# UW-RoboSoccer/tsid_control

Hardware: AMD Instinct MI355X
Metric: env-steps/sec (whole node) (higher is better)
Workload: dtype f64

## Files before the change

tsid_control_amd/csrc/tsidb_api.hip:

```cpp
#include "../../include/tsidb.h"
#include "tsidb_common.hpp"
#include "tsidb_sim.hpp"
#include "tsidb_tick.hpp"
#include "tsidb_policy.hpp"

#include <cmath>
#include <cstdio>
#include <cstring>
#include <string>
#include <vector>

using namespace tsidb;

template <typename T>
struct WalkArgs {
  const T *coef; const int *side; const int *nsteps; const T *rest; const T *com; int K;
  T t_now; const T *t_off; T Tstep, t_start, omega, z0, dz;
  const T *frames; T *foot_ref; T *contact_ref; uint8_t *cact; T *com_ref;
  const int *ncon; const int *con; int *latch; unsigned long long fgeoms0, fgeoms1; T td_frac; const double *t_dev;
};
template <typename T>
__device__ __forceinline__ void walk_update_env(const WalkArgs<T> &wa, int e, int r) {
  const T *coef = wa.coef, *rest = wa.rest, *com = wa.com, *t_off = wa.t_off, *frames = wa.frames;
  const int *side = wa.side, *nsteps = wa.nsteps, *ncon = wa.ncon, *con = wa.con;
// ... 170 lines not shown
  for (int b = 0; b < (MULTI ? B : 1); b++) {
    const DevModel<T> *mq = mp;
    if constexpr (MULTI) {
      asm volatile("" : "+s"(mq), "+s"(qpos), "+s"(qvel), "+s"(qacc_ws), "+s"(env_params), "+s"(terrain), "+s"(motor_tau) : : "memory");
      asm volatile("" : "+s"(qacc), "+s"(ncon), "+s"(con), "+s"(info) : : "memory");
      if constexpr (XF) asm volatile("" : "+s"(xfrc) : : "memory");
      if constexpr (RO) asm volatile("" : "+s"(ro.con_force), "+s"(ro.con_frame), "+s"(ro.con_pos), "+s"(ro.act_force), "+s"(ro.foot_grf) : : "memory");
      if constexpr (SE) asm volatile("" : "+s"(ro.sens) : : "memory");
      if constexpr (CT) asm volatile("" : "+s"(ctrl) : : "memory");
    }
    SimOut<T> roe{};
    if constexpr (RO) {
      roe.con_force = ro.con_force ? ro.con_force + E * MAXCON * 6 : nullptr;
      roe.con_frame = ro.con_frame ? ro.con_frame + E * MAXCON * 9 : nullptr;
      roe.con_pos = ro.con_pos ? ro.con_pos + E * MAXCON * 4 : nullptr;
      roe.act_force = ro.act_force ? ro.act_force + E * NA : nullptr;
      roe.foot_grf = ro.foot_grf ? ro.foot_grf + E * 12 : nullptr;
      roe.foot_body[0] = ro.foot_body[0]; roe.foot_body[1] = ro.foot_body[1];
    }
    if constexpr (SE) roe.sens = ro.sens + E * NSENS * mq->nsite;
    const size_t slot = (size_t)((ring.slots >> (4 * b)) & 15ull);
    const T *q_tsid = ring.q ? ring.q + slot * (size_t)n * NQ : nullptr, *v_tsid = ring.v ? ring.v + slot * (size_t)n * NV : nullptr;
    bool skip;
    {
      T chk = 0, big = 0;
      if (lane < NQ) { big += fabs(qpos[E * NQ + lane]); chk += q_tsid ? fabs(q_tsid[E * NQ + lane]) : T(0); }
      if (lane < NV) { big += fabs(qvel[E * NV + lane]); chk += fabs(qacc_ws[E * NV + lane]) + (v_tsid ? fabs(v_tsid[E * NV + lane]) : T(0)); }
      if (lane < NA && motor_tau) chk += fabs(motor_tau[E * NA + lane]);
      if constexpr (XF) for (int i = lane; i < NB * 6; i += WAVE) chk += fabs(xfrc[E * NB * 6 + i]);
      if constexpr (CT) { if (lane < NA) chk += fabs(ctrl[E * NA + lane]); }
      big = wave_sum(big);
      skip = __ballot(!(chk <= Eps<T>::inf)) || !(big <= T(SIM_STATE_BOUND));
      if (skip && wv == 0) {
        if (lane == 0) {
          if (info) { info[E * 4 + 2] = 0; info[E * 4 + 3] = 4; }
          if (ncon) ncon[e] = 0;
        }
        if (con && lane < MAXCON) con[E * MAXCON + lane] = -1;
        if constexpr (RO) sim_readouts_zero(roe, lane);
        if constexpr (SE) sim_sensors_zero(*mq, roe.sens, lane);
      }
    }
    if (!skip)
      sim_step_env<T, NW, XF, RO, SE, CT>(*mq, L, lane, wv, q_tsid ? q_tsid + E * NQ : nullptr, v_tsid ? v_tsid + E * NV : nullptr, qpos + E * NQ, qvel + E * NV, qacc_ws + E * NV,
                          env_params ? env_params + E * 8 : nullptr, terrain ? terrain + E * 20 : nullptr, XF ? xfrc + E * NB * 6 : nullptr,
                          motor_tau ? motor_tau + E * NA : nullptr, qacc ? qacc + E * NV : nullptr, ncon ? ncon + e : nullptr, con ? con + E * MAXCON : nullptr,
                          info ? info + E * 4 : nullptr, roe, CT ? ctrl + E * NA : nullptr, ctrl_mode);
    if constexpr (MULTI) __syncthreads();
  }
}

template <typename T>
__global__ __launch_bounds__(WAVE) void k_rbd(const DevModel<T> *__restrict__ mp, int n, const T *q, const T *v, T *M, T *hb,
                                              T *Jcom, T *Jf, T *oMf, T *com) {
  __shared__ TickLds<T> L;
  const int lane = threadIdx.x;
  if ((int)blockIdx.x >= n) return;
  const int e = env_of_block(blockIdx.x, n);
  const size_t E = (size_t)e;
  if (lane < NQ) L.qs[lane] = q[E * NQ + lane];
  if (lane < NV) L.vs[lane] = v[E * NV + lane];
  __syncthreads();
  rbd_terms<T>(*mp, L, lane);
  for (int i = lane; i < NV * NV; i += WAVE) M[E * NV * NV + i] = L.Dyn[(i / NV) * LDD + i % NV];
  if (lane < NV) hb[E * NV + lane] = L.h[lane];
  for (int i = lane; i < 3 * NV; i += WAVE) Jcom[E * 3 * NV + i] = L.k.Jcom[(i / NV) * LDF + i % NV];
  for (int i = lane; i < 12 * NV; i += WAVE) Jf[E * 12 * NV + i] = L.k.Jf[(i / NV) * LDF + i % NV];
// ... 505 lines not shown
  if ((int)ct[8] != CONDIM) throw std::string("model blob: contact dimension differs from this library's");
  const double *dmp = b.f64("mj_damping", NV), *ar = b.f64("mj_act_range", NA * 4);
  bool anyd = false;
  for (int i = 0; i < NV; i++) { m.mj_damping[i] = (T)dmp[i]; anyd |= dmp[i] != 0.0; }
  if (anyd != EULERDAMP) throw std::string("model blob: joint damping differs from what this library was built for");
  for (int i = 0; i < NA * 4; i++) {
    const double lim = sizeof(T) == 8 ? 1e300 : 1e30;
    m.act_range[i / 4][i % 4] = (T)(ar[i] > lim ? lim : (ar[i] < -lim ? -lim : ar[i]));
  }
  for (int i = 0; i < 7; i++) m.opt[i] = (T)op[i];
  m.opt[0] = (T)P[P_DT];
  m.opt[6] = sizeof(T) == 8 ? (T)1e-9 : (T)2e-6;
  for (int i = 0; i < 12; i++) m.contact[i] = (T)ct[i];
  const uint32_t nvert = h->blob.count("mj_hull_vert") / 3;
  m.hull_x = (const T *)h->d_hull;
  m.hull_y = m.hull_x + nvert;
  m.hull_z = m.hull_y + nvert;
  {
    const uint32_t np2 = b.count("mj_pairs");
    if (np2 % 2 || np2 / 2 > MAXPAIR) throw std::string("model blob: too many candidate body pairs");
    const int *pp = b.i32("mj_pairs", 0);
    m.npair = (int)(np2 / 2);
    for (int k = 0; k < m.npair; k++) {
      m.pair_a[k] = pp[2 * k]; m.pair_b[k] = pp[2 * k + 1];
      if (pp[2 * k] < 0 || pp[2 * k] >= NG || pp[2 * k + 1] < 0 || pp[2 * k + 1] >= NG) throw std::string("model blob: bad geom pair");
    }
    const double *hc = b.f64("mj_hull_center", NG * 3), *hb = b.f64("mj_hull_box", NG * 6);
    for (int i = 0; i < NG * 3; i++) m.hcen[i / 3][i % 3] = (T)hc[i];
    for (int i = 0; i < NG * 6; i++) m.hbox[i / 6][i % 6] = (T)hb[i];
    if (sizeof(T) == 4) for (int j = 0; j < NG; j++) for (int i = 3; i < 6; i++) m.hbox[j][i] = m.hbox[j][i] * (T)1.00001 + (T)1e-7;
  }
  memcpy(m.chunk_adr, b.i32("mj_chunk_adr", NG + 1), sizeof m.chunk_adr);
  m.chunk_box = (const T *)h->d_box;
  m.hull_eadr = h->d_eadr;
  m.hull_edge = h->d_edge;
  m.nsite = h->n_sites;
  for (int s = 0; s < h->n_sites; s++) {
    m.site_body[s] = h->site_body[s];
    for (int i = 0; i < 3; i++) m.site_pos[s][i] = (T)h->site_pos[s][i];
    for (int i = 0; i < 9; i++) m.site_R[s][i] = (T)h->site_R[s][i];
  }
}

static void validate_geometry(const Blob &b) {
  if constexpr (!TOPO_HAS_SIM) return;
  const int *ha = b.i32("mj_hull_adr", NG + 1), *ca = b.i32("mj_chunk_adr", NG + 1);
  const int64_t nvert = b.count("mj_hull_vert") / 3, nchunk = b.count("mj_chunk_box") / 6, nedge = b.count("mj_hull_edge");
  if (b.count("mj_hull_vert") % 3 || b.count("mj_chunk_box") % 6) throw std::string("model blob: hull vertex / chunk box sections are not whole records");
// ... 615 lines not shown
  need_refs(h);
  if (!q || !v || !tau || !dv || !f || !status) throw std::string("tsidb_tick_walk: null buffer");
  launch_tick(h, q, v, tau, dv, f, status, obs, obs_ld, frames, info, (hipStream_t)stream, nullptr, nullptr, walk, q_snapshot, v_snapshot);
  GUARD_END
}

int tsidb_rbd_terms(tsidb_handle h, const void *q, const void *v, void *M, void *hbias, void *Jcom, void *Jf, void *oMf,
                    void *com, void *stream) {
  GUARD_BEGIN
  if (!q || !v || !M || !hbias || !Jcom || !Jf || !oMf || !com) throw std::string("tsidb_rbd_terms: null buffer");
  hipStream_t s = (hipStream_t)stream;
  h->note_stream(s);
  with_dtype(h->dtype, [&](auto t) {
    using T = decltype(t);
    hipLaunchKernelGGL(k_rbd<T>, dim3(h->num_envs), dim3(WAVE), 0, s, (const DevModel<T> *)h->d_model, h->num_envs, (const T *)q,
                       (const T *)v, (T *)M, (T *)hbias, (T *)Jcom, (T *)Jf, (T *)oMf, (T *)com);
  });
  HIP_OK(hipGetLastError());
  GUARD_END
}

#ifdef TSIDB_STAMPS
int tsidb_debug_stamps(unsigned long long *out, int n) {
  return (int)hipMemcpyFromSymbol(out, HIP_SYMBOL(g_stamp), sizeof(unsigned long long) * 32 * (size_t)n);
}
#endif

int tsidb_dims(int *out9) {
  if (!out9) return -1;
  const int d[9] = {NJ, NQ, NV, NA, NB, TOPO_HAS_SIM, NG, CONDIM, TOPO_EULERDAMP};
  for (int i = 0; i < 9; i++) out9[i] = d[i];
  return 0;
}

int tsidb_lds_bytes(int dtype, int which) {
  return with_dtype(dtype, [&](auto t) { return which == 0 ? (int)sizeof(TickLds<decltype(t)>) : (int)sizeof(SimLds<decltype(t)>); });
}

}
```

tsid_control_amd/csrc/tsidb_common.hpp:

```cpp
#pragma once
#include <hip/hip_runtime.h>
#include <stdint.h>

#ifdef TSIDB_STAMPS
__device__ unsigned long long g_stamp[8192][32];
#define TSIDB_STAMP(k) do { if (threadIdx.x == 0 && blockIdx.x < 8192) g_stamp[blockIdx.x][k] = __builtin_amdgcn_s_memtime(); } while (0)
#define TSIDB_LAP_INIT() unsigned long long lap_t_ = __builtin_amdgcn_s_memtime()
#define TSIDB_LAP(k) do { unsigned long long n_ = __builtin_amdgcn_s_memtime(); if (threadIdx.x == 0 && blockIdx.x < 8192) g_stamp[blockIdx.x][k] += n_ - lap_t_; lap_t_ = n_; } while (0)
#define TSIDB_LAP_ZERO(k) do { if (threadIdx.x == 0 && blockIdx.x < 8192) g_stamp[blockIdx.x][k] = 0; } while (0)
#else
#define TSIDB_STAMP(k) do { } while (0)
#define TSIDB_LAP_INIT() do { } while (0)
#define TSIDB_LAP(k) do { } while (0)
#define TSIDB_LAP_ZERO(k) do { } while (0)
#endif

#ifndef TSIDB_TOPOLOGY_HEADER
#define TSIDB_TOPOLOGY_HEADER "tsidb_topology.hpp"
#endif
#include TSIDB_TOPOLOGY_HEADER

namespace tsidb {

constexpr int NJ = TOPO_NJ;
constexpr int NQ = TOPO_NQ;
constexpr int NV = TOPO_NV;
constexpr int NA = TOPO_NA;
constexpr int NB = TOPO_NB;
// ... 50 lines not shown
  int mj_last[NB];
  int mj_up[3][NB];
  int mj_chain[NB][8];
  int mj_maxdepth;
  T mj_pos[NB][3], mj_R[NB][9];
  T mj_inertia[NB][10];
  T mj_armature[NV], mj_frictionloss[NV], mj_dof_invw0[NV], mj_body_invw0[NB][2];
  int mj_act_dof[NA];
  T mj_act_kp[NA], mj_act_kv[NA];
  int mj_ctrl_qidx[NA];
  int tsid2sim[NA];
  int geom_body[NG];
  int hull_adr[NG + 1];
  T rbound[NG][4];
  T mj_damping[NV];
  T act_range[NA][4];
  T opt[7];
  T contact[12];
  T meaninertia;
  const T *hull_x, *hull_y, *hull_z;
  int chunk_adr[NG + 1];
  const T *chunk_box;
  const int *hull_eadr, *hull_edge;
  int npair, pair_a[MAXPAIR], pair_b[MAXPAIR];
  T hcen[NG][3], hbox[NG][6];
  int nsite, site_body[MAXSITE];
  T site_pos[MAXSITE][3], site_R[MAXSITE][9];
};

__device__ __forceinline__ unsigned long long plan_hash(unsigned long long seed, unsigned long long env, unsigned long long episode) {
  unsigned long long x = seed ^ (env * 0x9E3779B97F4A7C15ull) ^ (episode * 0xD1B54A32D192ED03ull);
  x += 0x9E3779B97F4A7C15ull;
  x = (x ^ (x >> 30)) * 0xBF58476D1CE4E5B9ull;
  x = (x ^ (x >> 27)) * 0x94D049BB133111EBull;
  return x ^ (x >> 31);
}

template <typename T> __device__ __forceinline__ void cross3(const T *a, const T *b, T *c) {
  T x = a[1] * b[2] - a[2] * b[1], y = a[2] * b[0] - a[0] * b[2], z = a[0] * b[1] - a[1] * b[0];
  c[0] = x; c[1] = y; c[2] = z;
}
template <typename T> __device__ __forceinline__ T dot3(const T *a, const T *b) { return a[0] * b[0] + a[1] * b[1] + a[2] * b[2]; }
template <typename T> __device__ __forceinline__ void mat3vec(const T *R, const T *v, T *o) {
  T x = R[0] * v[0] + R[1] * v[1] + R[2] * v[2];
  T y = R[3] * v[0] + R[4] * v[1] + R[5] * v[2];
  T z = R[6] * v[0] + R[7] * v[1] + R[8] * v[2];
  o[0] = x; o[1] = y; o[2] = z;
// ... 334 lines not shown
```

tsid_control_amd/csrc/tsidb_sim.hpp:

```cpp
#pragma once
#include "tsidb_common.hpp"
#include "tsidb_tick.hpp"

namespace tsidb {

constexpr int LDM = 27;
constexpr int NEWTON_INCR_MAX = 8;

template <typename T>
struct Floor {
  T n[3], t1[3], t2[3], d;
};

template <typename T>
struct SimLds {
  Floor<T> fl;
  T S[NV][6];
  union {
    struct { T V[NB][6], A[NB][6], f[NB][6], Yc[NB][10]; };
    struct {
      T K[NB][21];
      T hn[MAXHH][3];
      int hb1[MAXHH];
    };
// ... 326 lines not shown
      }
    }
  }
#pragma unroll
  for (int k = 0; k < K; k++) {
    T wxr[3];
    cross3(tw[k] + 3, L.cr[c], wxr);
    const T u[3] = {tw[k][0] + wxr[0], tw[k][1] + wxr[1], tw[k][2] + wxr[2]};
    const T un = dot3(n, u), u1 = dot3(t1, u), u2 = dot3(t2, u);
    out[k][0] = un + mu * u1; out[k][1] = un - mu * u1; out[k][2] = un + mu * u2; out[k][3] = un - mu * u2;
    if constexpr (CONDIM > 3) {
      const T ut = m.contact[9] * dot3(n, tw[k] + 3);
      out[k][4] = un + ut; out[k][5] = un - ut;
    }
  }
}

template <typename T> __device__ __forceinline__ T terrain_h(const T *terr, T X, T Y) {
  const T u = terr[0] * X + terr[1] * Y;
  const int cell = (int)floor((u - terr[2]) * terr[3]) & 15;
  return terr[4 + cell];
}

template <typename T, bool TERR>
__device__ __forceinline__ int hull_argmin(const DevModel<T> &m, int lane, int b, T r6, T r7, T r8, T pz, T tie, const T *terr,
                                           const T *Rw, T px, T py, T hmax_all, T &zmin_out) {
  const T INF = Eps<T>::inf;
  const int v0 = m.hull_adr[b], v1 = m.hull_adr[b + 1];
  const int c0 = m.chunk_adr[b], nch = m.chunk_adr[b + 1] - c0;
  T zlb = INF;
  if (lane < nch) {
    const T *bx = m.chunk_box + 6 * (c0 + lane);
    zlb = r6 * bx[0] + r7 * bx[1] + r8 * bx[2] + pz - (fabs(r6) * bx[3] + fabs(r7) * bx[4] + fabs(r8) * bx[5]);
    zlb -= fabs(zlb) * T(4) * Eps<T>::v;
    if constexpr (TERR) {
      const T a0 = terr[0] * Rw[0] + terr[1] * Rw[3], a1 = terr[0] * Rw[1] + terr[1] * Rw[4], a2 = terr[0] * Rw[2] + terr[1] * Rw[5];
      const T uc = a0 * bx[0] + a1 * bx[1] + a2 * bx[2] + terr[0] * px + terr[1] * py;
      const T ext = fabs(a0) * bx[3] + fabs(a1) * bx[4] + fabs(a2) * bx[5] + T(1e-6);
      const int k0 = (int)floor((uc - ext - terr[2]) * terr[3]), k1 = (int)floor((uc + ext - terr[2]) * terr[3]);
      T hm = hmax_all;
      if (k1 - k0 < 15) {
        hm = terr[4 + (k0 & 15)];
        for (int k = k0 + 1; k <= k1; k++) { const T hk = terr[4 + (k & 15)]; hm = hk > hm ? hk : hm; }
      }
      zlb -= hm;
    }
  }
  auto vert_val = [&](int i) -> T {
    const T x = m.hull_x[i], y = m.hull_y[i], z = m.hull_z[i];
    T val = r6 * x + r7 * y + r8 * z + pz;
    if constexpr (TERR) val -= terrain_h(terr, Rw[0] * x + Rw[1] * y + Rw[2] * z + px, Rw[3] * x + Rw[4] * y + Rw[5] * z + py);
    return val;
  };
  unsigned long long scanned = 0;
  T zmin = INF;
// ... 59 lines not shown
  const T d5 = -dot3(ab, c), d6 = -dot3(ac, c);
  if (d6 >= 0 && d5 <= d6) { q[0] = c[0]; q[1] = c[1]; q[2] = c[2]; return dot3(q, q); }
  const T vb = d5 * d2 - d1 * d6;
  if (vb <= 0 && d2 >= 0 && d6 <= 0) {
    const T t = d2 / (d2 - d6);
#pragma unroll
    for (int i = 0; i < 3; i++) q[i] = a[i] + t * ac[i];
    return dot3(q, q);
  }
  const T va = d3 * d6 - d5 * d4;
  if (va <= 0 && (d4 - d3) >= 0 && (d5 - d6) >= 0) {
    const T t = (d4 - d3) / ((d4 - d3) + (d5 - d6));
#pragma unroll
    for (int i = 0; i < 3; i++) q[i] = b[i] + t * (c[i] - b[i]);
    return dot3(q, q);
  }
  const T den = T(1) / (va + vb + vc), v = vb * den, w = vc * den;
#pragma unroll
  for (int i = 0; i < 3; i++) q[i] = a[i] + ab[i] * v + ac[i] * w;
  return dot3(q, q);
}

template <typename T>
__device__ __forceinline__ bool mpr_penetration(const DevModel<T> &m, const SimLds<T> &L, int lane, int a, int b, T margin, T &depth, T *dir_out, T *pos) {
  const T TOL = sizeof(T) == 8 ? T(1e-10) : T(2e-6), TIE = sizeof(T) == 8 ? T(1e-12) : T(1e-7);
  const T TINY2 = sizeof(T) == 8 ? T(1e-30) : T(1e-20), SIDE = sizeof(T) == 8 ? T(1e-14) : T(1e-9);
  constexpr int MAXIT = 64;
  const int ba = m.geom_body[a], bb = m.geom_body[b];
  const T *Ra = L.R[ba], *Rb = L.R[bb], *pa = L.p[ba], *pb = L.p[bb];
  auto wvert = [&](const T *R, const T *p, int i, T *w) {
    const T v[3] = {m.hull_x[i], m.hull_y[i], m.hull_z[i]};
    mat3vec(R, v, w);
    w[0] += p[0]; w[1] += p[1]; w[2] += p[2];
  };
  auto support = [&](const T *d, T *v, int &ia, int &ib) {
    T ra[3], rb[3], zz, wa[3], wb[3];
    mat3Tvec(Ra, d, ra);
    mat3Tvec(Rb, d, rb);
    ia = hull_argmin<T, false>(m, lane, a, -ra[0], -ra[1], -ra[2], T(0), TIE, nullptr, nullptr, T(0), T(0), T(0), zz);
    ib = hull_argmin<T, false>(m, lane, b, rb[0], rb[1], rb[2], T(0), TIE, nullptr, nullptr, T(0), T(0), T(0), zz);
    wvert(Ra, pa, ia, wa);
    wvert(Rb, pb, ib, wb);
    v[0] = wa[0] - wb[0]; v[1] = wa[1] - wb[1]; v[2] = wa[2] - wb[2];
    if (margin != 0) {
      v[0] += margin * d[0]; v[1] += margin * d[1]; v[2] += margin * d[2];
    }
  };
  T ca[3], cb[3], v0[3], v1[3], v2[3], v3[3], v4[3], dir[3], e1[3], e2[3];
  int i1a = 0, i1b = 0, i2a = 0, i2b = 0, i3a = 0, i3b = 0, i4a = 0, i4b = 0;
  mat3vec(Ra, m.hcen[a], ca);
  mat3vec(Rb, m.hcen[b], cb);
#pragma unroll
  for (int i = 0; i < 3; i++) { ca[i] += pa[i]; cb[i] += pb[i]; v0[i] = ca[i] - cb[i]; }
  if (dot3(v0, v0) < TINY2) { v0[0] = sizeof(T) == 8 ? T(1e-10) : T(1e-6); v0[1] = 0; v0[2] = 0; }
#pragma unroll
  for (int i = 0; i < 3; i++) dir[i] = -v0[i];
  normalize3(dir);
  support(dir, v1, i1a, i1b);
  if (dot3(v1, dir) <= 0) return false;
  cross3(v0, v1, dir);
  if (dot3(dir, dir) < TINY2) {
    const T d1 = sqrt(dot3(v1, v1));
    if (!(d1 > 0)) return false;
// ... 117 lines not shown
#pragma unroll
  for (int i = 0; i < 3; i++) { p1[i] = bw[0] * ca[i]; p2[i] = bw[0] * cb[i]; }
  wvert(Ra, pa, i1a, wa); wvert(Rb, pb, i1b, wb);
#pragma unroll
  for (int i = 0; i < 3; i++) { p1[i] += bw[1] * wa[i]; p2[i] += bw[1] * wb[i]; }
  wvert(Ra, pa, i2a, wa); wvert(Rb, pb, i2b, wb);
#pragma unroll
  for (int i = 0; i < 3; i++) { p1[i] += bw[2] * wa[i]; p2[i] += bw[2] * wb[i]; }
  wvert(Ra, pa, i3a, wa); wvert(Rb, pb, i3b, wb);
#pragma unroll
  for (int i = 0; i < 3; i++) { p1[i] += bw[3] * wa[i]; p2[i] += bw[3] * wb[i]; }
#pragma unroll
  for (int i = 0; i < 3; i++) pos[i] = T(0.5) * (p1[i] + p2[i]) / sum;
  return true;
}

template <typename T>
__device__ __forceinline__ bool spheres_overlap(const SimLds<T> &L, int a, int b, T margin) {
  const T d[3] = {L.scen[a][0] - L.scen[b][0], L.scen[a][1] - L.scen[b][1], L.scen[a][2] - L.scen[b][2]};
  const T rr = L.scen[a][3] + L.scen[b][3] + margin;
  return !(dot3(d, d) > rr * rr);
}
template <typename T>
__device__ __forceinline__ bool boxes_may_touch(const DevModel<T> &m, const SimLds<T> &L, int a, int b, T margin) {
  const int ba = m.geom_body[a], bb = m.geom_body[b];
  const T *Ra = L.R[ba], *Rb = L.R[bb];
  T ca[3], cb[3], d[3];
  mat3vec(Ra, m.hbox[a], ca);
  mat3vec(Rb, m.hbox[b], cb);
#pragma unroll
  for (int i = 0; i < 3; i++) d[i] = (cb[i] + L.p[bb][i]) - (ca[i] + L.p[ba][i]);
  const T hm = T(0.5) * margin;
  const T ha[3] = {m.hbox[a][3] + hm, m.hbox[a][4] + hm, m.hbox[a][5] + hm}, hb[3] = {m.hbox[b][3] + hm, m.hbox[b][4] + hm, m.hbox[b][5] + hm};
  T Rm[3][3], A[3][3], t[3];
#pragma unroll
  for (int i = 0; i < 3; i++) {
    t[i] = Ra[i] * d[0] + Ra[3 + i] * d[1] + Ra[6 + i] * d[2];
#pragma unroll
    for (int j = 0; j < 3; j++) {
      Rm[i][j] = Ra[i] * Rb[j] + Ra[3 + i] * Rb[3 + j] + Ra[6 + i] * Rb[6 + j];
      A[i][j] = fabs(Rm[i][j]) + (sizeof(T) == 8 ? T(1e-12) : T(1e-6));
    }
  }
  bool sep = false;
#pragma unroll
  for (int i = 0; i < 3; i++) sep |= fabs(t[i]) > ha[i] + A[i][0] * hb[0] + A[i][1] * hb[1] + A[i][2] * hb[2];
#pragma unroll
  for (int j = 0; j < 3; j++)
// ... 280 lines not shown
#pragma unroll
        for (int i = 0; i < 6; i++) a[i] += L.S[5 + c][i] * qa;
      }
    }
    T *o = sens + NSENS * lane;
    T r[3], t[3], acc[3], al[3], Rw[9];
#pragma unroll
    for (int i = 0; i < 3; i++) r[i] = o[i] - L.qpos[i];
    quat_to_R(o[4], o[5], o[6], o[3], Rw);
    cross3(a + 3, r, t);
#pragma unroll
    for (int i = 0; i < 3; i++) acc[i] = o[19 + i] + (a[i] + t[i]);
    mat3Tvec(Rw, acc, al);
#pragma unroll
    for (int i = 0; i < 3; i++) o[19 + i] = al[i];
  }
}

template <typename T> __device__ __forceinline__ void sim_sensors_zero(const DevModel<T> &m, T *sens, int lane) {
  for (int i = lane; i < NSENS * m.nsite; i += WAVE) sens[i] = 0;
}

enum { CTRL_POSITION = 1, CTRL_MOTOR = 2, CTRL_RESIDUAL = 3 };
template <typename T, int NW, bool XF, bool RO, bool SE = false, bool CT = false>
__device__ __forceinline__ void sim_step_env(const DevModel<T> &m, SimLds<T> &L, int lane, int wv, const T *q_tsid, const T *v_tsid, T *qpos_g, T *qvel_g,
                             T *qacc_ws_g, const T *envp, const T *terr_g, const T *xfrc, const T *motor_tau, T *qacc_out, int *ncon_out,
                             int *con_out, int *info, const SimOut<T> &ro, const T *ctrl = nullptr, int ctrl_mode = 0) {
  const T mscale = envp ? envp[0] : T(1);
  Floor<T> &fl = L.fl;
  if (lane == 0) {
    fl.n[0] = envp ? envp[2] : T(0); fl.n[1] = envp ? envp[3] : T(0); fl.n[2] = envp ? envp[4] : T(1);
    fl.d = envp ? envp[5] : T(0);
    T t[3] = {0, 0, 0};
    if (fabs(fl.n[1]) < T(0.5)) t[1] = 1; else t[2] = 1;
    const T dn = dot3(fl.n, t);
    T nn = 0;
#pragma unroll
    for (int i = 0; i < 3; i++) { fl.t1[i] = t[i] - dn * fl.n[i]; nn += fl.t1[i] * fl.t1[i]; }
    nn = T(1) / sqrt(nn);
#pragma unroll
    for (int i = 0; i < 3; i++) fl.t1[i] *= nn;
    cross3(fl.n, fl.t1, fl.t2);
  }
  const T gz = m.opt[1];
  const T INF = Eps<T>::inf;
  const T MINVAL = T(1e-15);
  const bool quirks = m.params[P_QUIRKS] != 0;

  TSIDB_STAMP(16);
  if (lane < NQ) {
    T val = qpos_g[lane];
    if (q_tsid) {
      if (lane < 3) val = q_tsid[lane];
      else if (lane < 7) val = quirks ? q_tsid[lane] : (lane == 3 ? q_tsid[6] : q_tsid[lane - 1]);
    }
    L.qpos[lane] = val;
  }
  if (lane < NV) {
    T val = qvel_g[lane];
    if (q_tsid && v_tsid && !quirks && lane < 6) {
      if (lane < 3) {
        const T x = q_tsid[3], y = q_tsid[4], z = q_tsid[5], w = q_tsid[6];
        const T r0 = lane == 0 ? 1 - 2 * (y * y + z * z) : lane == 1 ? 2 * (x * y + w * z) : 2 * (x * z - w * y);
        const T r1 = lane == 0 ? 2 * (x * y - w * z) : lane == 1 ? 1 - 2 * (x * x + z * z) : 2 * (y * z + w * x);
        const T r2 = lane == 0 ? 2 * (x * z + w * y) : lane == 1 ? 2 * (y * z - w * x) : 1 - 2 * (x * x + y * y);
        val = r0 * v_tsid[0] + r1 * v_tsid[1] + r2 * v_tsid[2];
      } else {
        val = v_tsid[lane];
      }
    }
    L.qvel[lane] = val;
  }
  T myctrl_ = (lane < NA && q_tsid) ? q_tsid[m.mj_ctrl_qidx[lane]] : T(0);
  if constexpr (CT) {
    if (lane < NA) myctrl_ = (ctrl_mode == CTRL_RESIDUAL && !motor_tau) ? myctrl_ + ctrl[lane] : ctrl[lane];
  }
  const T myctrl = myctrl_;
  for (int i = lane; i < NV * LDM; i += WAVE) L.M[i] = 0;
  __syncthreads();
  const T Oz = L.qpos[2];

  T Rb[9], pb[3], Vb[6], Ab[6], Sb[6], qd = 0;
  const int up0 = lane < NB ? m.mj_up[0][lane] : -1, up1 = lane < NB ? m.mj_up[1][lane] : -1,
            up2 = lane < NB ? m.mj_up[2][lane] : -1;
  const unsigned bodyanc = lane < NB ? m.mj_anc[lane] : 0u;
  if (lane < NB) L.anc[lane] = bodyanc;
#pragma unroll
  for (int i = 0; i < 6; i++) { Vb[i] = 0; Ab[i] = 0; Sb[i] = 0; }
#pragma unroll
  for (int i = 0; i < 3; i++) pb[i] = 0;
#pragma unroll
  for (int i = 0; i < 9; i++) Rb[i] = 0;
  if (lane == 0) {
    quat_to_R(L.qpos[4], L.qpos[5], L.qpos[6], L.qpos[3], Rb);
#pragma unroll
    for (int k = 0; k < 3; k++) {
// ... 176 lines not shown
  TSIDB_STAMP(17);
  T arow[NV];
  T qas = 0;
  int fail = 0;
  T *park = &L.cfv[0][0];
  if (w_dyn) {
#pragma unroll
    for (int j = 0; j < NV; j++) arow[j] = lane < NV ? L.M[lane * LDM + j] : T(0);
    bool spd;
    qas = chol26_solve<T, false>(arow, qfs, lane, spd);
    fail = spd ? 0 : 1;
    if (lane < NV) { park[lane] = qas; park[NV + lane] = qfs; }
  }

  TSIDB_STAMP(18);
  int ncon = 0, nfl = 0, cfail = 0;
  bool hh_cross = false;
  if (w_col) {
  if (has_terr) {
    if (lane < 20) L.terr[lane] = terr_g[lane];
    wsync<NW>();
  }
  const bool pm_rule = m.params[P_PLANE_MESH] != 0;
  for (unsigned long long bm = cand_geoms; bm; bm &= bm - 1) {
    const int g = __ffsll((long long)bm) - 1, b = m.geom_body[g];
    const T *Rb = L.R[b];
    const T r6 = fl.n[0] * Rb[0] + fl.n[1] * Rb[3] + fl.n[2] * Rb[6];
    const T r7 = fl.n[0] * Rb[1] + fl.n[1] * Rb[4] + fl.n[2] * Rb[7];
    const T r8 = fl.n[0] * Rb[2] + fl.n[1] * Rb[5] + fl.n[2] * Rb[8];
    const T pz = dot3(fl.n, L.p[b]) + nO;
    const int v0 = m.hull_adr[g];
    T zmin;
    const int best = has_terr ? hull_argmin<T, true>(m, lane, g, r6, r7, r8, pz, tie_tol, L.terr, Rb, L.p[b][0] + Ow[0],
                                                     L.p[b][1] + Ow[1], hmax_all, zmin)
                              : hull_argmin<T, false>(m, lane, g, r6, r7, r8, pz, tie_tol, nullptr, nullptr, T(0), T(0), T(0), zmin);
    if (!(zmin <= margin)) continue;
    const int e0 = m.hull_eadr[best];
    int nnb = m.hull_eadr[best + 1] - e0;
    if (nnb > WAVE - 1) { nnb = WAVE - 1; cfail |= 16; }
    bool keep = false;
    T w[3] = {0, 0, 0}, wd = 0;
    int vid = best;
    if (lane <= nnb) {
      if (lane > 0) vid = v0 + m.hull_edge[e0 + lane - 1];
      const T vv[3] = {m.hull_x[vid], m.hull_y[vid], m.hull_z[vid]};
      mat3vec(Rb, vv, w);
      w[0] += L.p[b][0]; w[1] += L.p[b][1]; w[2] += L.p[b][2];
      wd = dot3(fl.n, w) + nO;
      if (has_terr) wd -= terrain_h(L.terr, w[0] + Ow[0], w[1] + Ow[1]);
      keep = lane == 0 || wd <= margin;
    }
    T cp[3] = {w[0] - T(0.5) * wd * fl.n[0], w[1] - T(0.5) * wd * fl.n[1], w[2] - T(0.5) * wd * fl.n[2]};
    if (pm_rule) {
      const T d3[3] = {cp[0] - rdlane(cp[0], 0), cp[1] - rdlane(cp[1], 0), cp[2] - rdlane(cp[2], 0)};
      const T thr = T(0.3) * m.rbound[g][3];
      const bool far = lane > 0 && keep && !(dot3(d3, d3) < thr * thr);
      const unsigned long long fm = __ballot(far);
      keep = lane == 0 || (far && __popcll(fm & ((1ull << lane) - 1ull)) < 3);
    }
    const unsigned long long mask = __ballot(keep);
    if (ncon + __popcll(mask) > MAXCON) cfail |= 8;
    const int slot = ncon + __popcll(mask & ((1ull << lane) - 1ull));
    if (keep && slot < MAXCON) {
      const T dist = wd;
      L.cbody[slot] = b;
      L.cgeom[slot] = g;
      L.cvert[slot] = vid - v0;
      L.cdist[slot] = dist;
#pragma unroll
      for (int i = 0; i < 3; i++) L.cr[slot][i] = cp[i];
#pragma unroll
      for (int d = 0; d < 7; d++) { const int a = m.mj_chain[b][d]; L.cchain[slot][d] = (unsigned char)(a > 0 ? a : 0); }
    }
    ncon += __popcll(mask);
    ncon = ncon > MAXCON ? MAXCON : ncon;
  }
  nfl = ncon;
  if (m.params[P_SELF_COLLISION] != 0) {
    if (lane < NG) {
      const int gb = m.geom_body[lane];
      T c[3];
      mat3vec(L.R[gb], m.rbound[lane], c);
      L.scen[lane][0] = c[0] + L.p[gb][0]; L.scen[lane][1] = c[1] + L.p[gb][1]; L.scen[lane][2] = c[2] + L.p[gb][2];
      L.scen[lane][3] = m.rbound[lane][3];
    }
    wsync<NW>();
    int nsph = 0, ncand = 0;
    bool over = false, over64 = false;
    auto box_pass = [&](int cnt) {
      const int k = lane < cnt ? L.pcand[lane] : 0;
      const bool may = lane < cnt && boxes_may_touch(m, L, m.pair_a[k], m.pair_b[k], margin);
      const unsigned long long mk = __ballot(may);
      const int pos = ncand + __popcll(mk & ((1ull << lane) - 1ull));
      if (may && pos < WAVE) L.fcand[pos] = k;
      ncand += __popcll(mk);
    };
    for (int k0 = 0; k0 < m.npair; k0 += WAVE) {
      const int k = k0 + lane;
      const bool may = k < m.npair && spheres_overlap(L, m.pair_a[k], m.pair_b[k], margin);
      const unsigned long long mk = __ballot(may);
      if (may) L.pcand[nsph + __popcll(mk & ((1ull << lane) - 1ull))] = k;
      nsph += __popcll(mk);
      if (nsph > WAVE) {
        wsync<NW>();
        box_pass(WAVE);
        const int rest = lane < nsph - WAVE ? L.pcand[WAVE + lane] : 0;
        wsync<NW>();
        if (lane < nsph - WAVE) L.pcand[lane] = rest;
        nsph -= WAVE;
        wsync<NW>();
      }
    }
    wsync<NW>();
    box_pass(nsph);
    if (ncand > WAVE) { ncand = WAVE; over64 = true; }
    wsync<NW>();
    for (int ci = 0; ci < ncand; ci++) {
      const int k = L.fcand[ci];
      const int ga = m.pair_a[k], gb = m.pair_b[k], a = m.geom_body[ga], b = m.geom_body[gb];
      T depth, dir[3], pos[3];
      if (!mpr_penetration(m, L, lane, ga, gb, margin, depth, dir, pos)) continue;
      if (ncon - nfl >= MAXHH || ncon >= MAXCON) { over = true; continue; }
      if (lane == 0) {
        L.cbody[ncon] = b;
        L.cgeom[ncon] = gb;
        L.cvert[ncon] = 0x8000 | ga;
        L.cdist[ncon] = margin - depth;
        L.hb1_s[ncon - nfl] = a;
#pragma unroll
        for (int i = 0; i < 3; i++) { L.cr[ncon][i] = pos[i]; L.hn_s[ncon - nfl][i] = dir[i]; }
      }
      if (!((bodyanc_of(m, b) >> a) & 1u) && !((bodyanc_of(m, a) >> b) & 1u)) hh_cross = true;
      ncon++;
    }
    if (over) cfail |= 8;
    if (over64) cfail |= 32;
  }
  }
  if constexpr (NW > 1) {
    if (wv == NW - 1 && lane == 0) { L.xch[0] = ncon; L.xch[1] = nfl; L.xch[2] = hh_cross ? 1 : 0; L.xch[3] = cfail; }
    __syncthreads();
    if (wv != 0) return;
    ncon = L.xch[0]; nfl = L.xch[1]; hh_cross = L.xch[2] != 0; cfail = L.xch[3];
  }
// ... 96 lines not shown
    for (int i = 0; i < NROWC; i++) rs.cjar[i] = cjar_s[i];
    rows_eval(rs, T(0), cc, gg, hh);
    T cost_s = wave_sum(cc);
    if (cost_w > cost_s) {
      qacc = qas;
      Ma = mulM(L, park, lane);
    } else {
      qacc = xw;
      rs.fjar = fjar_w;
#pragma unroll
      for (int i = 0; i < NROWC; i++) rs.cjar[i] = cjar_w[i];
    }

    TSIDB_STAMP(20);
    asm volatile("" ::: "memory");
    auto solver_tol = [&]() { asm volatile("" ::: "memory"); const T t0 = m.opt[2]; return t0 > 64 * Eps<T>::v ? t0 : 64 * Eps<T>::v; };
    T cost = 0;
    int iter = 0;
    bool have_fac = false;
    const unsigned long long gfirst = __ballot(lane < nfl && (lane == 0 || L.cbody[lane] != L.cbody[lane > 0 ? lane - 1 : 0]));
    const bool grouped = nfl > 2;
    unsigned prevbits = 0;
    TSIDB_LAP_ZERO(24); TSIDB_LAP_ZERO(25); TSIDB_LAP_ZERO(26); TSIDB_LAP_ZERO(27); TSIDB_LAP_ZERO(28);
    TSIDB_LAP_INIT();
    while (true) {
      rows_eval(rs, T(0), cc, gg, hh);
      const T gauss = wave_sum(lane < NV ? T(0.5) * (Ma - qfs) * (qacc - qas) : T(0));
      const T newcost = gauss + wave_sum(cc);
      T ff = 0;
      bool fact = false;
      if (rs.has_f) {
        const T f = rs.floss, r = rs.fR;
        if (rs.fjar <= -r * f) ff = f;
        else if (rs.fjar >= r * f) ff = -f;
        else { ff = -rs.fD * rs.fjar; fact = true; }
      }
      T Arow[6] = {0, 0, 0, 0, 0, 0};
      T tors_e = 0, tors_f = 0;
      if (rs.has_c) {
        T fr[NROWC];
        T fv[3] = {0, 0, 0};
        T cn[3], ct1[3], ct2[3];
        contact_frame(L, lane, nfl, cn, ct1, ct2);
        if constexpr (CONDIM > 3) {
          const T mut = m.contact[9];
          const bool a4 = rs.cjar[4] < 0, a5 = rs.cjar[5] < 0;
// ... 124 lines not shown
#pragma unroll
            for (int j = 0; j < 3; j++) {
              L.Wc[lane][sym_idx(i, 3 + j)] += tors_e * cn[i] * cn[j];
              if (j >= i) L.Wc[lane][sym_idx(3 + i, 3 + j)] += tors_e * (xn[i] * cn[j] + cn[i] * xn[j]) + tors_f * cn[i] * cn[j];
            }
        }
      }
      wsync<NW>();
      unsigned touched = 0;
      {
        for (unsigned long long gm = gfirst; gm; gm &= gm - 1) {
          const int cf = __ffsll((long long)gm) - 1;
          const unsigned long long rest = gm & (gm - 1);
          const int ce = rest ? __ffsll((long long)rest) - 1 : nfl;
          touched |= L.anc[L.cbody[cf]];
          if (lane < 21) {
            T acc = 0;
            for (int c = cf; c < ce; c++) acc += L.Wc[c][lane];
            L.Wc[cf][lane] = acc;
          }
        }
      }
      wsync<NW>();
      for (int id = lane; id < NB * 21; id += WAVE) {
        const int a = id / 21, e = id - 21 * a;
        T acc = 0;
        for (unsigned long long gm = gfirst; gm; gm &= gm - 1) {
          const int cf = __ffsll((long long)gm) - 1;
          if ((L.anc[L.cbody[cf]] >> a) & 1u) acc += L.Wc[cf][e];
        }
        L.K[a][e] = acc;
      }
      wsync<NW>();
      T Gk[6] = {0, 0, 0, 0, 0, 0};
      const bool mine = lane < NV && ((touched >> (lane < 6 ? 0 : lane - 5)) & 1u);
      if (mine) {
        const int k = lane, bk = k < 6 ? 0 : k - 5;
#pragma unroll
        for (int i = 0; i < 6; i++) {
          T sacc = 0;
#pragma unroll
          for (int j = 0; j < 6; j++) sacc += L.K[bk][sym_idx(i, j)] * L.S[k][j];
          Gk[i] = sacc;
        }
      }
      wsync<NW>();
      for (int i = lane; i < NV * LDM; i += WAVE) L.H[i] = L.M[i];
      wsync<NW>();
      if (mine) {
        const int k = lane, bk = k < 6 ? 0 : k - 5;
        int chn[7];
#pragma unroll
        for (int d = 0; d < 7; d++) chn[d] = m.mj_chain[bk][d];
#pragma unroll
        for (int d = 0; d < 7 + 6; d++) {
          const int i = d < 7 ? (chn[d < 7 ? d : 0] > 0 ? 5 + chn[d < 7 ? d : 0] : -1) : d - 7;
          if (i < 0 || i > k) continue;
          T val = 0;
#pragma unroll
          for (int e = 0; e < 6; e++) val += L.S[i][e] * Gk[e];
          const T hv = L.M[i * LDM + k] + val;
          L.H[i * LDM + k] = hv;
          L.H[k * LDM + i] = hv;
        }
      }
      wsync<NW>();
      if (fact) L.H[lane * LDM + lane] += rs.fD;
      wsync<NW>();
      for (int c = nfl; c < ncon; c++) {
        T A6[6];
#pragma unroll
        for (int e = 0; e < 6; e++) A6[e] = rdlane_dyn(Arow[e], c);
        T jk[3] = {0, 0, 0};
        if (lane < NV) {
          const int bk = lane < 6 ? 0 : lane - 5;
          const int sgn = (int)((L.anc[L.cbody[c]] >> bk) & 1u) - (int)((L.anc[L.hb1[c - nfl]] >> bk) & 1u);
          if (sgn != 0) {
            T wxr[3];
            cross3(&L.S[lane][3], L.cr[c], wxr);
#pragma unroll
            for (int i = 0; i < 3; i++) jk[i] = sgn > 0 ? L.S[lane][i] + wxr[i] : -(L.S[lane][i] + wxr[i]);
          }
          T *g = &L.K[0][0] + 5 * lane;
          g[0] = A6[0] * jk[0] + A6[1] * jk[1] + A6[2] * jk[2];
          g[1] = A6[1] * jk[0] + A6[3] * jk[1] + A6[4] * jk[2];
          g[2] = A6[2] * jk[0] + A6[4] * jk[1] + A6[5] * jk[2];
          if constexpr (CONDIM > 3) {
            const T *hn = L.hn[c - nfl];
            g[3] = hn[0] * jk[0] + hn[1] * jk[1] + hn[2] * jk[2];
// ... 131 lines not shown
```

Before: 18.36 million.

## Preload sim inputs, pack collision pairs, prefetch hull heads, fuse K accumulation

```diff
diff --git a/tsid_control_amd/csrc/tsidb_api.hip b/tsid_control_amd/csrc/tsidb_api.hip
--- a/tsid_control_amd/csrc/tsidb_api.hip
+++ b/tsid_control_amd/csrc/tsidb_api.hip
@@ -216,10 +216,13 @@
     const size_t slot = (size_t)((ring.slots >> (4 * b)) & 15ull);
     const T *q_tsid = ring.q ? ring.q + slot * (size_t)n * NQ : nullptr, *v_tsid = ring.v ? ring.v + slot * (size_t)n * NV : nullptr;
     bool skip;
+    SimIn<T> in{};
     {
       T chk = 0, big = 0;
-      if (lane < NQ) { big += fabs(qpos[E * NQ + lane]); chk += q_tsid ? fabs(q_tsid[E * NQ + lane]) : T(0); }
-      if (lane < NV) { big += fabs(qvel[E * NV + lane]); chk += fabs(qacc_ws[E * NV + lane]) + (v_tsid ? fabs(v_tsid[E * NV + lane]) : T(0)); }
+      if (lane < NQ) { in.qpos = qpos[E * NQ + lane]; if (q_tsid) in.qt = q_tsid[E * NQ + lane]; }
+      if (lane < NV) { in.qvel = qvel[E * NV + lane]; if (v_tsid) in.vt = v_tsid[E * NV + lane]; }
+      if (lane < NQ) { big += fabs(in.qpos); chk += q_tsid ? fabs(in.qt) : T(0); }
+      if (lane < NV) { big += fabs(in.qvel); chk += fabs(qacc_ws[E * NV + lane]) + (v_tsid ? fabs(in.vt) : T(0)); }
       if (lane < NA && motor_tau) chk += fabs(motor_tau[E * NA + lane]);
       if constexpr (XF) for (int i = lane; i < NB * 6; i += WAVE) chk += fabs(xfrc[E * NB * 6 + i]);
       if constexpr (CT) { if (lane < NA) chk += fabs(ctrl[E * NA + lane]); }
@@ -236,7 +239,7 @@
       }
     }
     if (!skip)
-      sim_step_env<T, NW, XF, RO, SE, CT>(*mq, L, lane, wv, q_tsid ? q_tsid + E * NQ : nullptr, v_tsid ? v_tsid + E * NV : nullptr, qpos + E * NQ, qvel + E * NV, qacc_ws + E * NV,
+      sim_step_env<T, NW, XF, RO, SE, CT>(*mq, L, lane, wv, in, q_tsid ? q_tsid + E * NQ : nullptr, v_tsid ? v_tsid + E * NV : nullptr, qpos + E * NQ, qvel + E * NV, qacc_ws + E * NV,
                           env_params ? env_params + E * 8 : nullptr, terrain ? terrain + E * 20 : nullptr, XF ? xfrc + E * NB * 6 : nullptr,
                           motor_tau ? motor_tau + E * NA : nullptr, qacc ? qacc + E * NV : nullptr, ncon ? ncon + e : nullptr, con ? con + E * MAXCON : nullptr,
                           info ? info + E * 4 : nullptr, roe, CT ? ctrl + E * NA : nullptr, ctrl_mode);
@@ -788,8 +791,8 @@
     const int *pp = b.i32("mj_pairs", 0);
     m.npair = (int)(np2 / 2);
     for (int k = 0; k < m.npair; k++) {
-      m.pair_a[k] = pp[2 * k]; m.pair_b[k] = pp[2 * k + 1];
       if (pp[2 * k] < 0 || pp[2 * k] >= NG || pp[2 * k + 1] < 0 || pp[2 * k + 1] >= NG) throw std::string("model blob: bad geom pair");
+      m.pair_pk[k] = (unsigned)pp[2 * k] | (unsigned)pp[2 * k + 1] << 8 | (unsigned)m.geom_body[pp[2 * k]] << 16 | (unsigned)m.geom_body[pp[2 * k + 1]] << 24;
     }
     const double *hc = b.f64("mj_hull_center", NG * 3), *hb = b.f64("mj_hull_box", NG * 6);
     for (int i = 0; i < NG * 3; i++) m.hcen[i / 3][i % 3] = (T)hc[i];
@@ -1451,7 +1454,7 @@
 
 #ifdef TSIDB_STAMPS
 int tsidb_debug_stamps(unsigned long long *out, int n) {
-  return (int)hipMemcpyFromSymbol(out, HIP_SYMBOL(g_stamp), sizeof(unsigned long long) * 32 * (size_t)n);
+  return (int)hipMemcpyFromSymbol(out, HIP_SYMBOL(g_stamp), sizeof(unsigned long long) * NSTAMP * (size_t)n);
 }
 #endif
 
diff --git a/tsid_control_amd/csrc/tsidb_common.hpp b/tsid_control_amd/csrc/tsidb_common.hpp
--- a/tsid_control_amd/csrc/tsidb_common.hpp
+++ b/tsid_control_amd/csrc/tsidb_common.hpp
@@ -3,7 +3,8 @@
 #include <stdint.h>
 
 #ifdef TSIDB_STAMPS
-__device__ unsigned long long g_stamp[8192][32];
+constexpr int NSTAMP = 48;
+__device__ unsigned long long g_stamp[8192][NSTAMP];
 #define TSIDB_STAMP(k) do { if (threadIdx.x == 0 && blockIdx.x < 8192) g_stamp[blockIdx.x][k] = __builtin_amdgcn_s_memtime(); } while (0)
 #define TSIDB_LAP_INIT() unsigned long long lap_t_ = __builtin_amdgcn_s_memtime()
 #define TSIDB_LAP(k) do { unsigned long long n_ = __builtin_amdgcn_s_memtime(); if (threadIdx.x == 0 && blockIdx.x < 8192) g_stamp[blockIdx.x][k] += n_ - lap_t_; lap_t_ = n_; } while (0)
@@ -100,7 +101,8 @@
   int chunk_adr[NG + 1];
   const T *chunk_box;
   const int *hull_eadr, *hull_edge;
-  int npair, pair_a[MAXPAIR], pair_b[MAXPAIR];
+  int npair;
+  unsigned pair_pk[MAXPAIR];
   T hcen[NG][3], hbox[NG][6];
   int nsite, site_body[MAXSITE];
   T site_pos[MAXSITE][3], site_R[MAXSITE][9];
diff --git a/tsid_control_amd/csrc/tsidb_sim.hpp b/tsid_control_amd/csrc/tsidb_sim.hpp
--- a/tsid_control_amd/csrc/tsidb_sim.hpp
+++ b/tsid_control_amd/csrc/tsidb_sim.hpp
@@ -372,15 +372,30 @@
   return terr[4 + cell];
 }
 
+template <typename T> struct HullHead { int v0, v1, nch; T bx[6]; };
+template <typename T> __device__ __forceinline__ HullHead<T> hull_head(const DevModel<T> &m, int lane, int b) {
+  HullHead<T> h;
+  h.v0 = m.hull_adr[b]; h.v1 = m.hull_adr[b + 1];
+  const int c0 = m.chunk_adr[b];
+  h.nch = m.chunk_adr[b + 1] - c0;
+#pragma unroll
+  for (int i = 0; i < 6; i++) h.bx[i] = 0;
+  if (lane < h.nch) {
+    const T *bx = m.chunk_box + 6 * (c0 + lane);
+#pragma unroll
+    for (int i = 0; i < 6; i++) h.bx[i] = bx[i];
+  }
+  return h;
+}
+
 template <typename T, bool TERR>
-__device__ __forceinline__ int hull_argmin(const DevModel<T> &m, int lane, int b, T r6, T r7, T r8, T pz, T tie, const T *terr,
+__device__ __forceinline__ int hull_argmin(const DevModel<T> &m, int lane, const HullHead<T> &hd, T r6, T r7, T r8, T pz, T tie, const T *terr,
                                            const T *Rw, T px, T py, T hmax_all, T &zmin_out) {
   const T INF = Eps<T>::inf;
-  const int v0 = m.hull_adr[b], v1 = m.hull_adr[b + 1];
-  const int c0 = m.chunk_adr[b], nch = m.chunk_adr[b + 1] - c0;
+  const int v0 = hd.v0, v1 = hd.v1, nch = hd.nch;
   T zlb = INF;
   if (lane < nch) {
-    const T *bx = m.chunk_box + 6 * (c0 + lane);
+    const T *bx = hd.bx;
     zlb = r6 * bx[0] + r7 * bx[1] + r8 * bx[2] + pz - (fabs(r6) * bx[3] + fabs(r7) * bx[4] + fabs(r8) * bx[5]);
     zlb -= fabs(zlb) * T(4) * Eps<T>::v;
     if constexpr (TERR) {
@@ -486,11 +501,10 @@
 }
 
 template <typename T>
-__device__ __forceinline__ bool mpr_penetration(const DevModel<T> &m, const SimLds<T> &L, int lane, int a, int b, T margin, T &depth, T *dir_out, T *pos) {
+__device__ __forceinline__ bool mpr_penetration(const DevModel<T> &m, const SimLds<T> &L, int lane, int a, int b, int ba, int bb, T margin, T &depth, T *dir_out, T *pos) {
   const T TOL = sizeof(T) == 8 ? T(1e-10) : T(2e-6), TIE = sizeof(T) == 8 ? T(1e-12) : T(1e-7);
   const T TINY2 = sizeof(T) == 8 ? T(1e-30) : T(1e-20), SIDE = sizeof(T) == 8 ? T(1e-14) : T(1e-9);
   constexpr int MAXIT = 64;
-  const int ba = m.geom_body[a], bb = m.geom_body[b];
   const T *Ra = L.R[ba], *Rb = L.R[bb], *pa = L.p[ba], *pb = L.p[bb];
   auto wvert = [&](const T *R, const T *p, int i, T *w) {
     const T v[3] = {m.hull_x[i], m.hull_y[i], m.hull_z[i]};
@@ -501,8 +515,8 @@
     T ra[3], rb[3], zz, wa[3], wb[3];
     mat3Tvec(Ra, d, ra);
     mat3Tvec(Rb, d, rb);
-    ia = hull_argmin<T, false>(m, lane, a, -ra[0], -ra[1], -ra[2], T(0), TIE, nullptr, nullptr, T(0), T(0), T(0), zz);
-    ib = hull_argmin<T, false>(m, lane, b, rb[0], rb[1], rb[2], T(0), TIE, nullptr, nullptr, T(0), T(0), T(0), zz);
+    ia = hull_argmin<T, false>(m, lane, hull_head(m, lane, a), -ra[0], -ra[1], -ra[2], T(0), TIE, nullptr, nullptr, T(0), T(0), T(0), zz);
+    ib = hull_argmin<T, false>(m, lane, hull_head(m, lane, b), rb[0], rb[1], rb[2], T(0), TIE, nullptr, nullptr, T(0), T(0), T(0), zz);
     wvert(Ra, pa, ia, wa);
     wvert(Rb, pb, ib, wb);
     v[0] = wa[0] - wb[0]; v[1] = wa[1] - wb[1]; v[2] = wa[2] - wb[2];
@@ -666,8 +680,7 @@
   return !(dot3(d, d) > rr * rr);
 }
 template <typename T>
-__device__ __forceinline__ bool boxes_may_touch(const DevModel<T> &m, const SimLds<T> &L, int a, int b, T margin) {
-  const int ba = m.geom_body[a], bb = m.geom_body[b];
+__device__ __forceinline__ bool boxes_may_touch(const DevModel<T> &m, const SimLds<T> &L, int a, int b, int ba, int bb, T margin) {
   const T *Ra = L.R[ba], *Rb = L.R[bb];
   T ca[3], cb[3], d[3];
   mat3vec(Ra, m.hbox[a], ca);
@@ -994,8 +1007,9 @@
 }
 
 enum { CTRL_POSITION = 1, CTRL_MOTOR = 2, CTRL_RESIDUAL = 3 };
+template <typename T> struct SimIn { T qpos, qvel, qt, vt; };
 template <typename T, int NW, bool XF, bool RO, bool SE = false, bool CT = false>
-__device__ __forceinline__ void sim_step_env(const DevModel<T> &m, SimLds<T> &L, int lane, int wv, const T *q_tsid, const T *v_tsid, T *qpos_g, T *qvel_g,
+__device__ __forceinline__ void sim_step_env(const DevModel<T> &m, SimLds<T> &L, int lane, int wv, const SimIn<T> &in, const T *q_tsid, const T *v_tsid, T *qpos_g, T *qvel_g,
                              T *qacc_ws_g, const T *envp, const T *terr_g, const T *xfrc, const T *motor_tau, T *qacc_out, int *ncon_out,
                              int *con_out, int *info, const SimOut<T> &ro, const T *ctrl = nullptr, int ctrl_mode = 0) {
   const T mscale = envp ? envp[0] : T(1);
@@ -1020,30 +1034,32 @@
   const bool quirks = m.params[P_QUIRKS] != 0;
 
   TSIDB_STAMP(16);
-  if (lane < NQ) {
-    T val = qpos_g[lane];
+  {
+    const T qt_wxyz = __shfl(in.qt, lane == 3 ? 6 : (lane > 0 ? lane - 1 : 0), WAVE);
+    T val = in.qpos;
     if (q_tsid) {
-      if (lane < 3) val = q_tsid[lane];
-      else if (lane < 7) val = quirks ? q_tsid[lane] : (lane == 3 ? q_tsid[6] : q_tsid[lane - 1]);
-    }
-    L.qpos[lane] = val;
-  }
-  if (lane < NV) {
-    T val = qvel_g[lane];
+      if (lane < 3) val = in.qt;
+      else if (lane < 7) val = quirks ? in.qt : qt_wxyz;
+    }
+    if (lane < NQ) L.qpos[lane] = val;
+  }
+  {
+    T val = in.qvel;
     if (q_tsid && v_tsid && !quirks && lane < 6) {
       if (lane < 3) {
-        const T x = q_tsid[3], y = q_tsid[4], z = q_tsid[5], w = q_tsid[6];
+        const T x = rdlane(in.qt, 3), y = rdlane(in.qt, 4), z = rdlane(in.qt, 5), w = rdlane(in.qt, 6);
         const T r0 = lane == 0 ? 1 - 2 * (y * y + z * z) : lane == 1 ? 2 * (x * y + w * z) : 2 * (x * z - w * y);
         const T r1 = lane == 0 ? 2 * (x * y - w * z) : lane == 1 ? 1 - 2 * (x * x + z * z) : 2 * (y * z + w * x);
         const T r2 = lane == 0 ? 2 * (x * z + w * y) : lane == 1 ? 2 * (y * z - w * x) : 1 - 2 * (x * x + y * y);
-        val = r0 * v_tsid[0] + r1 * v_tsid[1] + r2 * v_tsid[2];
+        val = r0 * rdlane(in.vt, 0) + r1 * rdlane(in.vt, 1) + r2 * rdlane(in.vt, 2);
       } else {
-        val = v_tsid[lane];
-      }
-    }
-    L.qvel[lane] = val;
-  }
-  T myctrl_ = (lane < NA && q_tsid) ? q_tsid[m.mj_ctrl_qidx[lane]] : T(0);
+        val = in.vt;
+      }
+    }
+    if (lane < NV) L.qvel[lane] = val;
+  }
+  const T qt_act = __shfl(in.qt, lane < NA ? m.mj_ctrl_qidx[lane] : 0, WAVE);
+  T myctrl_ = (lane < NA && q_tsid) ? qt_act : T(0);
   if constexpr (CT) {
     if (lane < NA) myctrl_ = (ctrl_mode == CTRL_RESIDUAL && !motor_tau) ? myctrl_ + ctrl[lane] : ctrl[lane];
   }
@@ -1266,18 +1282,21 @@
     wsync<NW>();
   }
   const bool pm_rule = m.params[P_PLANE_MESH] != 0;
+  HullHead<T> head_next = hull_head(m, lane, cand_geoms ? __ffsll((long long)cand_geoms) - 1 : 0);
   for (unsigned long long bm = cand_geoms; bm; bm &= bm - 1) {
     const int g = __ffsll((long long)bm) - 1, b = m.geom_body[g];
+    const HullHead<T> head = head_next;
+    if (bm & (bm - 1)) head_next = hull_head(m, lane, __ffsll((long long)(bm & (bm - 1))) - 1);
     const T *Rb = L.R[b];
     const T r6 = fl.n[0] * Rb[0] + fl.n[1] * Rb[3] + fl.n[2] * Rb[6];
     const T r7 = fl.n[0] * Rb[1] + fl.n[1] * Rb[4] + fl.n[2] * Rb[7];
     const T r8 = fl.n[0] * Rb[2] + fl.n[1] * Rb[5] + fl.n[2] * Rb[8];
     const T pz = dot3(fl.n, L.p[b]) + nO;
-    const int v0 = m.hull_adr[g];
+    const int v0 = head.v0;
     T zmin;
-    const int best = has_terr ? hull_argmin<T, true>(m, lane, g, r6, r7, r8, pz, tie_tol, L.terr, Rb, L.p[b][0] + Ow[0],
+    const int best = has_terr ? hull_argmin<T, true>(m, lane, head, r6, r7, r8, pz, tie_tol, L.terr, Rb, L.p[b][0] + Ow[0],
                                                      L.p[b][1] + Ow[1], hmax_all, zmin)
-                              : hull_argmin<T, false>(m, lane, g, r6, r7, r8, pz, tie_tol, nullptr, nullptr, T(0), T(0), T(0), zmin);
+                              : hull_argmin<T, false>(m, lane, head, r6, r7, r8, pz, tie_tol, nullptr, nullptr, T(0), T(0), T(0), zmin);
     if (!(zmin <= margin)) continue;
     const int e0 = m.hull_eadr[best];
     int nnb = m.hull_eadr[best + 1] - e0;
@@ -1319,8 +1338,15 @@
     ncon += __popcll(mask);
     ncon = ncon > MAXCON ? MAXCON : ncon;
   }
+  TSIDB_STAMP(32);
   nfl = ncon;
   if (m.params[P_SELF_COLLISION] != 0) {
+    constexpr int PAIR_ROUNDS = MAXPAIR / WAVE;
+    constexpr bool PAIRS_AHEAD = PAIR_ROUNDS <= 4;
+    const int npair = m.npair;
+    unsigned pk[PAIRS_AHEAD ? PAIR_ROUNDS : 1];
+#pragma unroll
+    for (int r = 0; r < (PAIRS_AHEAD ? PAIR_ROUNDS : 1); r++) pk[r] = m.pair_pk[r * WAVE + lane];
     if (lane < NG) {
       const int gb = m.geom_body[lane];
       T c[3];
@@ -1329,21 +1355,21 @@
       L.scen[lane][3] = m.rbound[lane][3];
     }
     wsync<NW>();
+    TSIDB_STAMP(33);
     int nsph = 0, ncand = 0;
     bool over = false, over64 = false;
     auto box_pass = [&](int cnt) {
-      const int k = lane < cnt ? L.pcand[lane] : 0;
-      const bool may = lane < cnt && boxes_may_touch(m, L, m.pair_a[k], m.pair_b[k], margin);
+      const unsigned w = lane < cnt ? (unsigned)L.pcand[lane] : 0u;
+      const bool may = lane < cnt && boxes_may_touch(m, L, (int)(w & 255u), (int)((w >> 8) & 255u), (int)((w >> 16) & 255u), (int)(w >> 24), margin);
       const unsigned long long mk = __ballot(may);
       const int pos = ncand + __popcll(mk & ((1ull << lane) - 1ull));
-      if (may && pos < WAVE) L.fcand[pos] = k;
+      if (may && pos < WAVE) L.fcand[pos] = (int)w;
       ncand += __popcll(mk);
     };
-    for (int k0 = 0; k0 < m.npair; k0 += WAVE) {
-      const int k = k0 + lane;
-      const bool may = k < m.npair && spheres_overlap(L, m.pair_a[k], m.pair_b[k], margin);
+    auto sphere_round = [&](unsigned w, int k0) {
+      const bool may = k0 + lane < npair && spheres_overlap(L, (int)(w & 255u), (int)((w >> 8) & 255u), margin);
       const unsigned long long mk = __ballot(may);
-      if (may) L.pcand[nsph + __popcll(mk & ((1ull << lane) - 1ull))] = k;
+      if (may) L.pcand[nsph + __popcll(mk & ((1ull << lane) - 1ull))] = (int)w;
       nsph += __popcll(mk);
       if (nsph > WAVE) {
         wsync<NW>();
@@ -1354,16 +1380,30 @@
         nsph -= WAVE;
         wsync<NW>();
       }
+    };
+    if constexpr (PAIRS_AHEAD) {
+#pragma unroll
+      for (int r = 0; r < PAIR_ROUNDS; r++)
+        if (r * WAVE < npair) sphere_round(pk[r], r * WAVE);
+    } else {
+      unsigned cur = pk[0];
+      for (int k0 = 0; k0 < npair; k0 += WAVE) {
+        const unsigned nxt = k0 + WAVE < MAXPAIR ? m.pair_pk[k0 + WAVE + lane] : 0u;
+        sphere_round(cur, k0);
+        cur = nxt;
+      }
     }
     wsync<NW>();
+    TSIDB_STAMP(34);
     box_pass(nsph);
     if (ncand > WAVE) { ncand = WAVE; over64 = true; }
     wsync<NW>();
+    TSIDB_STAMP(35);
     for (int ci = 0; ci < ncand; ci++) {
-      const int k = L.fcand[ci];
-      const int ga = m.pair_a[k], gb = m.pair_b[k], a = m.geom_body[ga], b = m.geom_body[gb];
+      const unsigned w = (unsigned)L.fcand[ci];
+      const int ga = (int)(w & 255u), gb = (int)((w >> 8) & 255u), a = (int)((w >> 16) & 255u), b = (int)(w >> 24);
       T depth, dir[3], pos[3];
-      if (!mpr_penetration(m, L, lane, ga, gb, margin, depth, dir, pos)) continue;
+      if (!mpr_penetration(m, L, lane, ga, gb, a, b, margin, depth, dir, pos)) continue;
       if (ncon - nfl >= MAXHH || ncon >= MAXCON) { over = true; continue; }
       if (lane == 0) {
         L.cbody[ncon] = b;
@@ -1506,6 +1546,7 @@
     const bool grouped = nfl > 2;
     unsigned prevbits = 0;
     TSIDB_LAP_ZERO(24); TSIDB_LAP_ZERO(25); TSIDB_LAP_ZERO(26); TSIDB_LAP_ZERO(27); TSIDB_LAP_ZERO(28);
+    TSIDB_LAP_ZERO(36); TSIDB_LAP_ZERO(38); TSIDB_LAP_ZERO(39);
     TSIDB_LAP_INIT();
     while (true) {
       rows_eval(rs, T(0), cc, gg, hh);
@@ -1676,29 +1717,31 @@
         }
       }
       wsync<NW>();
-      for (int id = lane; id < NB * 21; id += WAVE) {
-        const int a = id / 21, e = id - 21 * a;
-        T acc = 0;
-        for (unsigned long long gm = gfirst; gm; gm &= gm - 1) {
-          const int cf = __ffsll((long long)gm) - 1;
-          if ((L.anc[L.cbody[cf]] >> a) & 1u) acc += L.Wc[cf][e];
-        }
-        L.K[a][e] = acc;
-      }
-      wsync<NW>();
+      TSIDB_LAP(36);
       T Gk[6] = {0, 0, 0, 0, 0, 0};
       const bool mine = lane < NV && ((touched >> (lane < 6 ? 0 : lane - 5)) & 1u);
       if (mine) {
         const int k = lane, bk = k < 6 ? 0 : k - 5;
+        T Kk[21];
+#pragma unroll
+        for (int e = 0; e < 21; e++) Kk[e] = 0;
+        for (unsigned long long gm = gfirst; gm; gm &= gm - 1) {
+          const int cf = __ffsll((long long)gm) - 1;
+          if ((L.anc[L.cbody[cf]] >> bk) & 1u) {
+#pragma unroll
+            for (int e = 0; e < 21; e++) Kk[e] += L.Wc[cf][e];
+          }
+        }
 #pragma unroll
         for (int i = 0; i < 6; i++) {
           T sacc = 0;
 #pragma unroll
-          for (int j = 0; j < 6; j++) sacc += L.K[bk][sym_idx(i, j)] * L.S[k][j];
+          for (int j = 0; j < 6; j++) sacc += Kk[sym_idx(i, j)] * L.S[k][j];
           Gk[i] = sacc;
         }
       }
       wsync<NW>();
+      TSIDB_LAP(38);
       for (int i = lane; i < NV * LDM; i += WAVE) L.H[i] = L.M[i];
       wsync<NW>();
       if (mine) {
@@ -1719,6 +1762,7 @@
         }
       }
       wsync<NW>();
+      TSIDB_LAP(39);
       if (fact) L.H[lane * LDM + lane] += rs.fD;
       wsync<NW>();
       for (int c = nfl; c < ncon; c++) {
```

New measurement: 18.67 million (median of 6 runs). 1.02x the previous value.
